# ontypehq/libfst

Hardware: AMD Instinct MI355X
Metric: strings/sec, compose_frozen_shortest_path_ambiguous len=64 batch=1M (higher is better)
Workload: dtype f64; 1 GPU; compose_frozen_shortest_path_ambiguous; semantics=eager, len=64, transducer_len=4096, branches=12, strings_per_gpu=1048576, global_batch=1048576, scaling_mode=weak: 1048576 strings per GPU per step, parallelism=dp1 (string shards, rhs replicated via RCCL broadcast)

## Files before the change

### libfst_amd/csrc/code_pull.hip

```cpp
#include <algorithm>

#include "pull_kernel_dispatch.hpp"

namespace fstamd {

namespace {
const void* pull_codes_kernel_for(const DeviceFst& rhs, uint32_t max_len, bool log = false) {
  const int rk = pull_rk(rhs, max_len);
  if (rk < 2) return nullptr;
  route_rk("eager", rk, rhs.rev, log);
  if (rk == 3) {
    const bool pack = pull_pack(rhs, max_len);
    if (log && std::getenv("FSTAMD_ROUTE_LOG"))
      std::fprintf(stderr, "[libfst_amd route] eager pull: packed cells %s\n", pack ? "on" : "off");
    if (pack) return pull_kernel_for<6, false, true>(rhs.rev);
  }
  switch (rk) {
    case 5: return pull_kernel_for<5, false, true>(rhs.rev);
    case 4: return pull_kernel_for<4, false, true>(rhs.rev);
    case 3: return pull_kernel_for<3, false, true>(rhs.rev);
    default: return pull_kernel_for<2, false, true>(rhs.rev);
  }
}
}

bool pull_codes_table(const DeviceFst& rhs, int semantics, uint32_t max_len, double* table) {
  if (semantics != 1 || !rhs.pull_ok || !pull_codes_kernel_for(rhs, max_len)) return false;
  const int rk = pull_rk(rhs, max_len);
  if (rk >= 4) {
    if (rhs.wtab_host.size() != kPullWtMax) return false;
    std::copy(rhs.wtab_host.begin(), rhs.wtab_host.end(), table);
  } else {
    for (uint32_t c = 0; c < 256; ++c) table[c] = (double)c * rhs.rev.winv;
  }
  return true;
}

int code_pull_waves_per_cu(const DeviceFst& rhs, uint32_t max_len) {
  int occ = 0;
  const void* k = pull_codes_kernel_for(rhs, max_len);
  if (!k || hipOccupancyMaxActiveBlocksPerMultiprocessor(&occ, k, 64, 0) != hipSuccess) occ = 1;
  return std::max(occ, 1);
}

hipError_t launch_eager_pull_codes(const DeviceFst& rhs, const ChainInput& in, uint32_t n_best,
                                   unsigned int* next_item, const EagerLaunch& lp,
                                   const BatchOutDev& out, uint32_t grid, hipStream_t stream) {
  const void* k = pull_codes_kernel_for(rhs, in.max_len, true);
  if (!k) return hipErrorInvalidValue;
  void* args[] = {(void*)&rhs.view, (void*)&rhs.rev, (void*)&in, (void*)&n_best,
                  (void*)&next_item, (void*)&lp, (void*)&out};
  return hipLaunchKernel(k, dim3(grid), dim3(64), args, 0, stream);
}

}
```

### libfst_amd/csrc/device_engine.hpp

```cpp
#pragma once

#include <hip/hip_runtime.h>

#include <atomic>
#include <condition_variable>
#include <cstdint>
#include <functional>
#include <mutex>
#include <new>
#include <vector>

#include "fst_core.hpp"

namespace fstamd {

class FrozenFst;

constexpr uint32_t kSpanMixed = 0xFFFFFFFEu;
constexpr uint32_t kSpanNone = 0xFFFFFFFFu;
constexpr uint32_t kRecPad = 16;
constexpr uint32_t kDeadLabel = 0xFFFFFFFFu;

struct RhsView {
  const uint2* span;
  const double* final_w;
  const uint32_t* il;
  const ArcRec* rec;
  const uint4* sspan;
  uint32_t num_states;
  uint32_t num_arcs;
  uint32_t start;
  uint32_t max_span;
  uint32_t jump_back;
  uint32_t jump_fwd;
  const uint4* sspan2;
};

constexpr uint32_t kRevPos = 0x1000u;
struct RevRec {
  uint32_t src;
  uint32_t y;
  double weight;
};
static_assert(sizeof(RevRec) == 16, "RevRec is one 16-byte load");
struct RevView {
  const uint4* rspan;
  const uint4* gtab;
  const RevRec* rrec;
  const uint32_t* rolab;
  uint32_t kp;
  uint32_t gsearch;
  uint32_t direct;
  const uint4* rrec32;
  const uint2* rrec8;
  const uint32_t* rlab;
  const uint2* rxrec;
  uint32_t nrec;
  const uint32_t* rrec4;
  uint32_t rbias8;
  double winv;
};
constexpr uint32_t kPullWt = 64;
constexpr uint32_t kPullWtMax = 256;
__host__ __device__ inline const double* rv_weight_table(const RevView& rv) {
  return reinterpret_cast<const double*>(rv.rrec4 + ((rv.nrec + 1u) & ~1u));
}
__host__ __device__ inline const uint32_t* rv_packed(const RevView& rv) {
  return rv.rrec4 + ((rv.nrec + 1u) & ~1u);
}
constexpr double kRec8WMax = 7.0;

struct DeviceFst {
  int dev = 0;
  uint8_t* blob = nullptr;
  size_t blob_size = 0;
  uint2* span = nullptr;
  double* final_w = nullptr;
  uint32_t* il = nullptr;
  ArcRec* rec = nullptr;
  uint4* sspan = nullptr;
  RhsView view{};
  bool has_eps = false;
  bool nonneg = true;
  bool nan = false;
  bool finite = true;
  uint8_t weight_type = 0;
  bool pull_ok = false;
  bool lazy_pull_ok = false;
  double int_wmax = -1.0;
  bool widx = false;
  uint32_t wt_n = 0;
  bool pack = false;
  bool byte_back = false;
  std::vector<double> wtab_host;
  mutable std::atomic<int> skip_tiny_lazy{0}, skip_tiny_eager{0};
  mutable std::atomic<int> tiny_lazy_256{0}, tiny_eager_256{0};
  mutable std::atomic<uint64_t> tiny_lazy_seen{0}, tiny_lazy_over{0};
  RevView rev{};
  void* rev_bufs[9] = {};
  uint32_t* band_il = nullptr;
  ArcRec* band_rec = nullptr;
  uint32_t band_sh = 0;
  bool band_ol_sorted = false;
  std::vector<uint32_t> perm;

  static DeviceFst* create(const FrozenFst& f, int dev);
  static DeviceFst* adopt(const void* d_blob, const FrozenFst& host_view, int dev);
  static void destroy(DeviceFst* d);
};

struct BatchOutDev {
  int32_t* status;
  uint32_t* path_len;
  uint64_t* path_off;
  double* final_w;
  uint32_t* out_il;
  uint32_t* out_ol;
  double* out_w;
  uint64_t arc_cap;
  unsigned long long* cursor;
  uint32_t* work;
  const uint64_t* slots = nullptr;
  uint32_t* host_ol = nullptr;
  union {
    double* host_w = nullptr;
    const struct TextOutDev* text;
    const struct LatticeOutDev* lattice;
  };
  int32_t* first_status = nullptr;
};

constexpr uint32_t kTextNotBytes = 0xFFFFFFFFu;
struct TextOutDev {
  uint8_t* host_text;
  uint32_t* nbytes;
  double* total_w;
};

struct LatItem {
  uint64_t spos, apos;
  uint32_t n, a;
  uint32_t pad[2];
};
static_assert(sizeof(LatItem) == 32, "two 16-B stores per item");
struct LatticeOutDev {
// ... 524 lines not shown
```

### libfst_amd/csrc/eager_pull.hip

```cpp
#include <algorithm>
#include <cmath>
#include <cstdio>
#include <cstdlib>
#include <cstring>
#include <unordered_map>
#include <vector>

#include "device_engine.hpp"
#include "host_fst.hpp"
#include "kernels/pull_window.hpp"
#include "pull_kernel_dispatch.hpp"

namespace fstamd {


void free_reverse_mirror(DeviceFst* d) {
  for (void*& p : d->rev_bufs) {
    if (p) (void)hipFree(p);
    p = nullptr;
  }
  d->rev = RevView{};
  d->pull_ok = false;
  d->widx = false;
  d->wt_n = 0;
  d->wtab_host.clear();
  d->pack = false;
}

bool build_reverse_mirror(DeviceFst* d, const FrozenFst& f) {
  d->pull_ok = false;
  d->lazy_pull_ok = false;
  if (std::getenv("FSTAMD_NO_PULL")) return true;
  if (d->has_eps || !d->nonneg || d->nan) return true;
  const uint32_t ns = f.num_states(), na = f.header().num_arcs;
  if (ns == 0 || ns >= (1u << 27)) return true;
  const StateEntry* se = f.states();
  const PackedArc* pa = f.arcs();
  const std::vector<uint32_t>& perm = d->perm;
  auto pid = [&](uint32_t s) { return perm.empty() ? s : perm[s]; };

  std::vector<uint8_t> jpos(na);
  std::vector<uint32_t> src(na);
  std::vector<uint32_t> indeg(ns + 1, 0);
  for (uint32_t s = 0; s < ns; ++s) {
    uint32_t run = se[s].arc_offset;
    for (uint32_t a = se[s].arc_offset; a < se[s].arc_offset + se[s].num_arcs; ++a) {
      if (a > se[s].arc_offset && pa[a].ilabel != pa[a - 1].ilabel) run = a;
      if (a - run >= 8) return true;
      jpos[a] = (uint8_t)(a - run);
      src[a] = pid(s);
      ++indeg[pid(pa[a].nextstate)];
    }
  }
  bool ol_ordered = true;
  for (uint32_t s = 0; s < ns && ol_ordered; ++s)
    for (uint32_t a = se[s].arc_offset; a < se[s].arc_offset + se[s].num_arcs && ol_ordered; ++a)
      for (uint32_t b = a - jpos[a]; b < a; ++b)
        if (pa[b].nextstate == pa[a].nextstate && pa[b].olabel > pa[a].olabel) {
          ol_ordered = false;
          break;
        }
  std::vector<uint32_t> ioff(ns + 1, 0);
  for (uint32_t t = 0; t < ns; ++t) ioff[t + 1] = ioff[t] + indeg[t];
  std::vector<uint32_t> in(na), fill(ioff.begin(), ioff.end() - 1);
  for (uint32_t a = 0; a < na; ++a) in[fill[pid(pa[a].nextstate)]++] = a;
  for (uint32_t t = 0; t < ns; ++t)
    std::sort(in.begin() + ioff[t], in.begin() + ioff[t + 1], [&](uint32_t x, uint32_t y) {
      if (pa[x].ilabel != pa[y].ilabel) return pa[x].ilabel < pa[y].ilabel;
      if (src[x] != src[y]) return src[x] < src[y];
      return jpos[x] < jpos[y];
    });
  struct Group { uint32_t t, label, first, n; };
  std::vector<Group> groups;
  for (uint32_t t = 0; t < ns; ++t)
    for (uint32_t i = ioff[t]; i < ioff[t + 1];) {
      uint32_t e = i + 1;
      while (e < ioff[t + 1] && pa[in[e]].ilabel == pa[in[i]].ilabel) ++e;
      groups.push_back(Group{t, pa[in[i]].ilabel, i, e - i});
      i = e;
// ... 126 lines not shown
  };
  std::vector<uint32_t> rrec4;
  uint32_t rbias8 = 0;
  int64_t dlo = 0, dhi = 0;
  if (!rrec8.empty() || widx) {
    for (size_t r = 0; r < rrec.size(); ++r) {
      if (rrec[r].src == 0xFFFFFFF8u) continue;
      const int64_t dl = (int64_t)rtgt[r] - (int64_t)(rrec[r].src >> 3);
      dlo = std::min(dlo, dl);
      dhi = std::max(dhi, dl);
    }
    if ((dhi - dlo) * 8 < 0xFFF0 && -dlo * 8 + 8 * (int64_t)kPullW <= 0xFFFF && byte_back) {
      rbias8 = (uint32_t)(-dlo * 8);
      rrec4.resize(rrec.size());
      for (size_t r = 0; r < rrec.size(); ++r) {
        const uint32_t y = rrec[r].y;
        if (rrec[r].src == 0xFFFFFFF8u) {
          rrec4[r] = 0xFFFF0000u;
        } else {
          const uint32_t low = (((y >> 17) & 7u) << 13) | (((y >> 13) & 15u) << 9) |
                               (((y >> 12) & 1u) << 8) | low_weight(rrec[r].weight);
          const int64_t dl = (int64_t)rtgt[r] - (int64_t)(rrec[r].src >> 3);
          rrec4[r] = ((uint32_t)((dl - dlo) * 8) << 16) | low;
        }
      }
    }
  }
  if (d->int_wmax >= 0.0) {
    rrec32.resize(rrec.size());
    for (size_t r = 0; r < rrec.size(); ++r)
      rrec32[r] = make_uint4(rrec[r].src, rrec[r].y, wsc(rrec[r].weight), rolab[r]);
  }
  bool pack = !rrec4.empty() && !widx && !rrec8.empty() && kp < 15 && rbias8 % 8 == 0;
  for (size_t g = 0; g < groups.size() && pack; ++g) pack = groups[g].label != 0xFFFFFFu;
  for (size_t r = 0; r < rrec4.size() && pack; ++r)
    pack = rrec4[r] == 0xFFFF0000u || (rrec4[r] >> 16) / 2 <= 252;
  pack = pack && pack_guards_fit((uint32_t)std::max<int64_t>(d->view.jump_back, -dlo),
                                 (uint32_t)std::max<int64_t>(d->view.jump_fwd, dhi), kPullW);
  if (pack) {
    const size_t n = rrec4.size();
    rrec4.resize(((n + 1) & ~(size_t)1) + n, 0xFFFF0000u);
    uint32_t* const rpk = rrec4.data() + ((n + 1) & ~(size_t)1);
    for (size_t r = 0; r < n; ++r) {
      const uint32_t v = rrec4[r];
      if (v == 0xFFFF0000u) {
        const size_t first = r - r % kp;
        rpk[r] = first < r && rrec4[first] != 0xFFFF0000u ? (rpk[first] & ~15u) | 15u : 15u;
      } else {
        rpk[r] = ((v >> 17) << 24) | ((v & 0xFFu) << 16) | (((v >> 13) & 7u) << 4) | ((v >> 9) & 15u);
      }
    }
  }
  d->pack = pack;
  if (rrec4.empty()) wtab.clear();
  if (!wtab.empty()) {
    d->wt_n = (uint32_t)wtab.size();
    wtab.resize(kPullWtMax, 0.0);
    d->wtab_host = wtab;
    rrec4.resize((rrec4.size() + 1) & ~(size_t)1, 0xFFFF0000u);
    const size_t at = rrec4.size();
    rrec4.resize(at + 2 * kPullWtMax);
    std::memcpy(rrec4.data() + at, wtab.data(), kPullWtMax * sizeof(double));
  }
  d->widx = !wtab.empty();
  auto up = [&](int i, const void* src_p, size_t bytes) -> bool {
    if (bytes == 0) bytes = 16;
    if (hipMalloc(&d->rev_bufs[i], bytes) != hipSuccess) return false;
    return hipMemcpy(d->rev_bufs[i], src_p, bytes, hipMemcpyHostToDevice) == hipSuccess;
  };
  const uint4 zero4 = make_uint4(0u, 0u, 0u, 0u);
  if (gtab.empty()) gtab.push_back(zero4);
  if (!up(0, rspan.data(), rspan.size() * sizeof(uint4)) ||
      !up(1, gtab.data(), gtab.size() * sizeof(uint4)) ||
      !up(2, rrec.data(), rrec.size() * sizeof(RevRec)) ||
      !up(3, rolab.data(), rolab.size() * sizeof(uint32_t)) ||
      (!rrec32.empty() && !up(4, rrec32.data(), rrec32.size() * sizeof(uint4))) ||
      (!rrec8.empty() && !up(5, rrec8.data(), rrec8.size() * sizeof(uint2))) ||
      (direct && (!up(6, rlab.data(), rlab.size() * sizeof(uint32_t)) ||
                  !up(7, rxrec.data(), rxrec.size() * sizeof(uint2)))) ||
      (!rrec4.empty() && !up(8, rrec4.data(), rrec4.size() * sizeof(uint32_t)))) {
    free_reverse_mirror(d);
    return false;
  }
  d->rev = RevView{(const uint4*)d->rev_bufs[0], (const uint4*)d->rev_bufs[1],
                   (const RevRec*)d->rev_bufs[2], (const uint32_t*)d->rev_bufs[3], kp, gsearch,
                   direct ? 1u : 0u, (const uint4*)d->rev_bufs[4], (const uint2*)d->rev_bufs[5],
                   (const uint32_t*)d->rev_bufs[6], (const uint2*)d->rev_bufs[7],
                   (uint32_t)(nblocks * kp), (const uint32_t*)d->rev_bufs[8], rbias8,
                   1.0 / wscale};
  d->byte_back = byte_back;
  d->pull_ok = true;
  d->lazy_pull_ok = ol_ordered && d->finite && !std::getenv("FSTAMD_NO_LAZY_PULL");
  return true;
}

bool pull_f32(const DeviceFst& rhs, uint32_t max_len) {
  return rhs.int_wmax >= 0.0 && rhs.rev.rrec32 && (double)max_len * rhs.int_wmax < 16777216.0;
}

int pull_waves_per_cu(const DeviceFst& rhs, uint32_t max_len) {
  int occ = 0;
  if (hipOccupancyMaxActiveBlocksPerMultiprocessor(&occ, pull_kernel_for<false>(rhs, max_len), 64, 0) !=
      hipSuccess)
    occ = 1;
  return std::max(occ, 1);
}
// ... 32 lines not shown
```

### libfst_amd/csrc/kernels/eager_pull.hpp

```cpp
#pragma once

#include <type_traits>

#include "device_common.hpp"
#include "eager_layered.hpp"
#include "eager_wave.hpp"
#include "eager_window.hpp"
#include "pull_window.hpp"

namespace fstamd {

constexpr uint32_t kPullAbsent = 0xFFFF0000u;
#ifdef FSTAMD_P_TIGHT_SELECT
constexpr bool kTightSelect = true;
#else
constexpr bool kTightSelect = false;
#endif
constexpr uint32_t kDistAbsent = 0x7F000000u;
template <typename DT>
__device__ __forceinline__ DT dist_inf() {
  if constexpr (sizeof(DT) == 4) return (DT)kDistAbsent;
  else return (DT)__builtin_huge_val();
}
template <typename DT>
__device__ __forceinline__ DT dist_min(DT a, DT b) {
  if constexpr (sizeof(DT) == 4) return min(a, b);
  else return fmin(a, b);
}


template <int W, bool F32 = false, int WT = kPullWt>
struct PullLds {
  static constexpr int kWords = W * 8 / 64;
  double d[W + 1];
  unsigned long long rk[W + 1];
  unsigned long long bits[kWords];
  uint4 pre[kWords];
  unsigned long long best;
  uint32_t bestp;
  ChaseJob job[kChaseBatch];
  double wt[WT];
};
template <int W>
struct PullLds<W, true> {
  static constexpr int kWords = W * 8 / 64;
  uint2 cell[W + 1];
  unsigned long long bits[kWords];
  uint4 pre[kWords];
  unsigned long long best;
  uint32_t bestp;
  ChaseJob job[kChaseBatch];
};

constexpr uint32_t kPackAbsent = 0x7F00FF80u;
constexpr uint32_t kPackNoRank = 0xFF80u;
constexpr uint32_t kPackPadM = 15u;
template <int W>
struct PullLdsPacked {
  static constexpr int kWords = W * 8 / 64;
  static constexpr int kCells = (int)pack_cells(W);
  static_assert(pack_guards_fit(kPackSpanMax, 0, W) && pack_guards_fit(0, kPackSpanMax, W),
                "packed cells: the guard bands hold every source of a window row");
  uint32_t cell[kCells];
  unsigned long long bits[kWords];
  uint4 pre[kWords];
  unsigned long long best;
  uint32_t bestp;
  ChaseJob job[kChaseBatch];
};
__device__ __forceinline__ uint32_t pack_candidate(uint32_t r, uint32_t c) {
  uint32_t cand;
  asm("v_mad_u32_u24 %0, %1, 1, %2" : "=v"(cand) : "v"(r), "v"(c));
  return cand;
}
__device__ __forceinline__ bool pack_counts(uint32_t cand) {
  return (cand & 0xFFFFu) < kPackNoRank && (cand & 15u) != kPackPadM;
}

template <int KP, typename DT>
__device__ __forceinline__ uint32_t tight_min(const DT (&nd)[KP], DT b, const uint32_t (&pk)[KP]) {
  uint32_t t[KP];
#pragma unroll
  for (int m = 0; m < KP; ++m) t[m] = nd[m] == b ? pk[m] : 0xFFFFFFFFu;
  uint32_t c = t[0];
#pragma unroll
  for (int m = 1; m < KP; m += 2) c = m + 1 < KP ? min(min(c, t[m]), t[m + 1]) : min(c, t[m]);
  return c;
}

template <typename T>
__device__ __forceinline__ const T* at_byte(const T* base, uint32_t byte_off) {
  return reinterpret_cast<const T*>(reinterpret_cast<const char*>(base) + byte_off);
}

template <int W>
__device__ __forceinline__ void pull_candidate(const PullLds<W>& S, const RevRec& r,
                                               uint32_t tmin8, uint32_t& pk, double& nd,
                                               uint32_t& rank_word) {
  const uint32_t off = min(r.src - tmin8, 8u * W);
  const double d = *reinterpret_cast<const double*>(reinterpret_cast<const char*>(S.d) + FB(off, 8 * (W + 1), 150));
  const uint32_t rw = *reinterpret_cast<const uint32_t*>(reinterpret_cast<const char*>(S.rk) + FB(off, 8 * (W + 1), 151));
  pk = rw | r.y | off;
  rank_word = rw;
  nd = d + r.weight;
}
template <int W, int WT>
__device__ __forceinline__ void pull_candidate(const PullLds<W, false, WT>& S, const uint32_t& r,
                                               uint32_t base8, uint32_t& pk, double& nd,
                                               uint32_t& rank_word) {
// ... 22 lines not shown
  const uint32_t off = min(r.x - tmin8, 8u * W);
  const uint2 c = *reinterpret_cast<const uint2*>(reinterpret_cast<const char*>(S.cell) + FB(off, 8 * (W + 1), 152));
  pk = c.y | r.y | off;
  rank_word = c.y;
  nd = c.x + rec8_weight(r.y);
}

template <int W>
__device__ __forceinline__ void pull_candidate(const PullLds<W, true>& S, const uint32_t& r,
                                               uint32_t base8, uint32_t& pk, uint32_t& nd,
                                               uint32_t& rank_word) {
  const uint32_t off = min(base8 - (r >> 16), 8u * W);
  const uint2 c = *reinterpret_cast<const uint2*>(reinterpret_cast<const char*>(S.cell) + FB(off, 8 * (W + 1), 152));
  pk = c.y | (r & 0xFFFFu);
  rank_word = c.y;
  nd = c.x + (r & 0xFFu);
}

__device__ __forceinline__ void pull_group(const RevView& rv, uint32_t lab, uint32_t t,
                                           uint32_t& rec0, uint32_t& nb) {
  const uint4 rs = rv.rspan[t];
  const bool hit = rs.z == lab && lab < kSpanMixed;
  rec0 = hit ? rs.x : 0u;
  nb = hit ? rs.y : 0u;
  if (rv.gsearch && __ballot(rs.z == kSpanMixed)) {
    if (rs.z == kSpanMixed) {
      uint32_t a = rs.x, b = rs.x + rs.y;
      for (uint32_t it = 0; it < rv.gsearch; ++it) {
        if (a < b) {
          const uint32_t mid = (a + b) >> 1;
          if (rv.gtab[mid].x < lab) a = mid + 1;
          else b = mid;
        }
      }
      if (a < rs.x + rs.y) {
        const uint4 g = rv.gtab[a];
        if (g.x == lab) {
          rec0 = g.y;
          nb = g.z;
        }
      }
    }
  }
}

template <int EW, int KP, bool DIRECT, int WAVES_PER_EU, int RK = 0, bool TEXT = false,
          bool CODES = false>
__global__ void __launch_bounds__(64, WAVES_PER_EU)
eager_pull_kernel(RhsView rhs, RevView rv, ChainInput in, uint32_t n_best,
                  unsigned int* next_item, EagerLaunch lp, BatchOutDev out) {
  constexpr int W = 64 * EW;
  constexpr bool F32 = RK != 0 && RK != 4 && RK != 5;
  constexpr bool REC4 = RK >= 3;
  constexpr bool PACK = RK == 6;
  static_assert(!PACK || (DIRECT && KP < (int)kPackPadM), "packed cells: direct layout, m = 15 is padding");
  static_assert(!CODES || (RK >= 2 && RK <= 6 && !TEXT), "weight codes: byte-weight records, label batches");
  constexpr int WT = RK == 5 ? (int)kPullWtMax : (int)kPullWt;
  using DT = typename std::conditional<F32, uint32_t, double>::type;
  using RT = typename std::conditional<
      REC4, uint32_t,
      typename std::conditional<RK == 2, uint2,
                                typename std::conditional<F32, uint4, RevRec>::type>::type>::type;
  constexpr uint32_t kRankShift = PACK ? 7 : REC4 ? 16 : 20;
  constexpr uint32_t kFirstShift = kRankShift - 3;
  constexpr uint32_t kMShift = kFirstShift - 4;
  using LdsT = typename std::conditional<PACK, PullLdsPacked<W>, PullLds<W, F32, WT>>::type;
  constexpr int kWords = LdsT::kWords;
  constexpr uint32_t kAbsent = PACK ? kPackNoRank : kPullAbsent;
  static_assert(KP <= 16, "m is 4 bits of the key");
  static_assert(W < 512, "8 * slot is 12 bits of the key, ranks 9 bits");
  __shared__ LdsT S;
  const uint32_t lane = threadIdx.x;
  const DT kInf = PACK ? (DT)(kPackAbsent >> 16) : dist_inf<DT>();
  const uint32_t* const rpk = PACK ? rv_packed(rv) : nullptr;
  auto set_cell = [&](uint32_t i, DT d, uint32_t rw) {
    if constexpr (PACK) {
      S.cell[FB(kPackGuardLo + i, LdsT::kCells, 153)] = ((uint32_t)d << 16) | rw;
    } else if constexpr (F32) {
      S.cell[FB(i, W + 1, 153)] = make_uint2(d, rw);
    } else {
      S.d[FB(i, W + 1, 154)] = d;
      S.rk[FB(i, W + 1, 155)] = rw;
    }
  };
  auto rec = [&](uint32_t r) -> RT {
    if constexpr (PACK) return rpk[r];
    else if constexpr (REC4) return rv.rrec4[r];
    else if constexpr (RK == 2) return rv.rrec8[r];
    else if constexpr (F32) return rv.rrec32[r];
    else return rv.rrec[r];
  };
  uint2* const slabs = lp.back_ws + (size_t)blockIdx.x * kChaseBatch * lp.back_cap;
  uint32_t njobs = 0;

  auto chase_batch = [&]() {
    wave_lds_sync();
    uint32_t maxL = 0;
    ChaseJob jb{};
    if (lane < njobs) {
      jb = S.job[FB(lane, kChaseBatch, 156)];
      maxL = jb.L;
    }
    maxL = __builtin_amdgcn_readfirstlane(__ockl_wfred_max_u32(maxL));
    const uint32_t* sl = reinterpret_cast<const uint32_t*>(slabs + (size_t)lane * lp.back_cap);
    const uint2* hdr = slabs + (size_t)lane * lp.back_cap + lp.back_cap / 2;
    uint32_t id = jb.id;
    uint32_t tcur = jb.pad;
    for (uint32_t t = 0; t < maxL; ++t) {
      if (lane < njobs && t < jb.L) {
        const uint32_t k = jb.L - 1 - t;
        uint32_t b;
        if constexpr (REC4) {
          const uint32_t v = reinterpret_cast<const uint8_t*>(sl)[FB(id, lp.back_cap, 60)];
          b = FB(v < (uint32_t)KP ? tcur * KP + v : rv.rxrec[tcur].x + v - KP, rv.nrec, 63);
        } else {
          b = FB(sl[FB(id, lp.back_cap, 60)], rv.nrec, 63);
        }
        const uint2 h = hdr[k];
        if constexpr (!TEXT)
          if (!out.host_ol) out.out_il[jb.o + k] = in.labels[jb.off + k];
        uint32_t src8;
        if constexpr (PACK) {
          const uint32_t r = rpk[b];
          out.out_ol[jb.o + k] = rv.rolab[b];
          if constexpr (CODES)
            reinterpret_cast<uint8_t*>(out.out_w)[jb.o + k] = (uint8_t)(r >> 16);
          else
// ... 60 lines not shown
    asm volatile("" : "+s"(w));
    return w != 0u;
  };

  if constexpr (PACK) {
#pragma unroll 1
    for (uint32_t i = lane; i < (uint32_t)LdsT::kCells; i += 64)
      S.cell[FB(i, LdsT::kCells, 153)] = kPackAbsent;
  } else {
#pragma unroll 1
  for (uint32_t i = lane; i < (uint32_t)W + 1; i += 64) set_cell(i, kInf, kAbsent);
  }
  if (lane < (uint32_t)kWords) S.bits[FB(lane, kWords, 157)] = 0;
  if constexpr (RK == 4 || RK == 5)
    for (uint32_t i = lane; i < (uint32_t)WT; i += 64) S.wt[i] = rv_weight_table(rv)[i];
  wave_lds_sync();
  uint32_t wlast = 0;

  for (;;) {
    uint32_t item = 0;
    if (lane == 0) item = atomicAdd(next_item, 1u);
    item = __builtin_amdgcn_readfirstlane(item);
    if (item >= num_items) break;
    const uint32_t si = __builtin_amdgcn_readfirstlane(lp.items ? lp.items[item] : item);
    uint32_t* const back = reinterpret_cast<uint32_t*>(slabs + (size_t)njobs * lp.back_cap);
    uint2* const hdr = slabs + (size_t)njobs * lp.back_cap + lp.back_cap / 2;
    const uint64_t off0 = in.offsets[si];
    const uint64_t off = ((uint64_t)__builtin_amdgcn_readfirstlane((uint32_t)(off0 >> 32)) << 32) |
                         __builtin_amdgcn_readfirstlane((uint32_t)off0);
    const uint32_t L = __builtin_amdgcn_readfirstlane((uint32_t)(in.offsets[si + 1] - off));

    if (rhs.start == kNoState || n_best != 1) {
      if (lane == 0)
        write_status(out, si, (rhs.start == kNoState || n_best == 0) ? kPathEmpty : kPathErrorN,
                     0, 0);
      continue;
    }
    const unsigned long long t0 = __builtin_amdgcn_s_memrealtime();

#pragma unroll 1
    for (uint32_t i = lane; i < wlast; i += 64) set_cell(i, kInf, kAbsent);
    wave_lds_sync();
    if (lane == 0) set_cell(0, (DT)w_one(), 0u);
    wave_lds_sync();
    uint32_t tmin = rhs.start, wk = 1, base = 0, n_cur = 1;
    uint32_t cmin = rhs.start, cmax = rhs.start;
    uint32_t tuples = 1, relax = 0;
    int32_t fail = F32 && L > in.max_len ? kPathOverflow : kPathOk;
    unsigned long long mykey = kMaxU64;
    uint32_t myp = kEmptyKey;
    double myfw = 0.0;

    uint32_t labs = 0;
    for (uint32_t k = 0; k < L && fail == kPathOk; ++k) {
      if ((k & 15u) == 0 && __builtin_amdgcn_s_memrealtime() - t0 > lp.wd_ticks) {
        fail = kPathInternal;
        break;
      }
      if constexpr (TEXT) {
        if ((k & 63u) == 0) labs = k + lane < L ? in.text[off + k + lane] + 1u : 0u;
      } else
      if ((k & 63u) == 0) labs = k + lane < L ? in.labels[off + k + lane] : 0u;
      const uint32_t lab = __builtin_amdgcn_readlane(labs, k & 63u);
      if (lab == kEpsilon) {
        fail = kPathUnsupported;
        break;
      }
      const uint32_t tn = pull_win_tn(cmin, rhs.jump_back);
      const uint32_t hi = pull_win_hi(cmax, rhs.jump_fwd, rhs.num_states);
      const uint32_t nbase = base + wk;
      if (pull_win_overflow(tn, hi, (uint32_t)W) || nbase + pull_win_wn(tn, hi) > lp.back_cap ||
          k >= lp.back_cap / 2) {
        fail = kPathOverflow;
        break;
      }
      const uint32_t wn = pull_win_wn(tn, hi);
      const uint32_t rows_n = pull_win_rows(wn);

      uint32_t fst[EW], bk[EW], bra[EW];
      DT bd[EW];
#pragma unroll
      for (int e = 0; e < EW; ++e) {
        fst[e] = kEmptyKey;
        bk[e] = kEmptyKey;
        bra[e] = 0;
        bd[e] = kInf;
        if ((uint32_t)e >= rows_n) continue;
        const uint32_t i = (uint32_t)e * 64 + lane;
        const uint32_t t = tn + i;
        uint32_t rec0, nb, xrec = 0;
        uint32_t tmin8 = tmin << 3;
        RT rr[KP];
        if constexpr (DIRECT) {
          const uint32_t rs = *at_byte(rv.rlab, t * 4u);
          if constexpr (PACK) {
            const uint32_t* const R = at_byte(rpk, t * (4u * KP));
#pragma unroll
            for (int m = 0; m < KP; ++m) rr[m] = R[m];
            __builtin_amdgcn_sched_barrier(0);
          }
          const bool hit = (rs & 0xFFFFFFu) == lab && lab < (PACK ? 0xFFFFFFu : kSpanMixed);
          if constexpr (PACK) tmin8 = hit ? pack_hit_base4(t, tmin, rv.rbias8 >> 1) : kPackMissBase4;
          else tmin8 = hit ? tmin8 : tmin8 + 0x80000000u;
          rec0 = t * KP;
          nb = hit ? rs >> 24 : 0u;
        } else {
          pull_group(rv, lab, t, rec0, nb);
        }
        if constexpr (REC4 && !PACK) tmin8 = (t << 3) - (tmin << 3) + rv.rbias8 + (tmin8 - (tmin << 3));
        if constexpr (!PACK) {
          const RT* R;
          if constexpr (REC4) R = at_byte(rv.rrec4, rec0 * 4u);
          else if constexpr (RK == 2) R = at_byte(rv.rrec8, rec0 * 8u);
          else if constexpr (F32) R = rv.rrec32 + rec0;
          else R = rv.rrec + rec0;
#pragma unroll
          for (int m = 0; m < KP; ++m) rr[m] = R[m];
        }
        uint32_t pk[KP], rw[KP];
        DT nd[KP];
        uint32_t f = kEmptyKey;
        DT b = kInf;
        uint32_t c = kEmptyKey;
        if constexpr (PACK) {
#pragma unroll
          for (int m = 0; m < KP; ++m) {
            const uint32_t off = pack_src_off4(tmin8, rr[m] >> 24);
            rw[m] = *reinterpret_cast<const uint32_t*>(reinterpret_cast<const char*>(S.cell) + FB(off, 4 * LdsT::kCells, 152));
          }
#pragma unroll
          for (int m = 0; m < KP; ++m) pk[m] = pack_candidate(rr[m], rw[m]);
// ... 24 lines not shown
            for (int m = 0; m < KP; ++m) c = min(c, nd[m] == b ? pk[m] : kEmptyKey);
          }
          if (want_work()) {
#pragma unroll
            for (int m = 0; m < KP; ++m) relax += (uint32_t)__popcll(__ballot(rw[m] < kPullAbsent));
          }
        }
        uint32_t ra = (REC4 ? 0u : rec0) + ((c >> kMShift) & 15u);
        if (__ballot(nb > 1)) {
          if constexpr (DIRECT) {
            const uint2 xr = nb > 1 ? rv.rxrec[t] : make_uint2(0u, nb);
            xrec = xr.x;
            nb = xr.y;
          }
          for (uint32_t x = 1;; ++x) {
            const bool act = nb > x;
            if (!__ballot(act)) break;
            const uint32_t rx = act ? (DIRECT ? xrec + (x - 1) * KP : rec0 + x * KP)
                                    : (DIRECT ? rhs.num_states * KP : 0u);
#pragma unroll
            for (int m = 0; m < KP; ++m) {
              if constexpr (PACK) {
                const uint32_t r2 = rec(rx + m);
                const uint32_t off = pack_src_off4(tmin8, r2 >> 24);
                const uint32_t cl = *reinterpret_cast<const uint32_t*>(reinterpret_cast<const char*>(S.cell) + FB(off, 4 * LdsT::kCells, 152));
                const uint32_t p2 = pack_candidate(r2, cl);
                if (act) {
                  f = min(f, p2 & 0xFFFFu);
                  if (p2 < c) {
                    c = p2;
                    ra = x * KP + m;
                  }
                }
                if (want_work()) relax += (uint32_t)__popcll(__ballot(act && pack_counts(p2)));
              } else {
                uint32_t p2, w2;
                DT n2;
                pull_candidate<W>(S, rec(rx + m), tmin8, p2, n2, w2);
                f = min(f, p2);
                if (n2 < b || (n2 == b && p2 < c)) {
                  b = n2;
                  c = p2;
                  ra = REC4 ? x * KP + m : rx + m;
                }
                if (want_work()) relax += (uint32_t)__popcll(__ballot(w2 < kPullAbsent));
              }
            }
          }
        }
        fst[e] = f;
        bd[e] = b;
        bk[e] = c;
        bra[e] = ra;
        if (f < kAbsent) {
          const uint32_t key = f >> kFirstShift;
          atomicOr(reinterpret_cast<uint32_t*>(S.bits) + FB(key >> 5, 2 * kWords, 158), 1u << (key & 31u));
        }
      }
      wave_lds_sync();

      const uint32_t nw = (n_cur * 8 + 63) / 64;
      unsigned long long word = 0;
      if (lane < nw) word = S.bits[FB(lane, kWords, 159)];
      const uint32_t pc = (uint32_t)__popcll(word);
      const uint32_t inc = wave_incl_scan_dpp(pc);
      const uint32_t n_next = __builtin_amdgcn_readlane(inc, 63);
      if (lane < nw) {
        S.pre[FB(lane, kWords, 160)] = make_uint4(inc - pc, (uint32_t)word,
                                 inc - pc + (uint32_t)__popc((uint32_t)word), (uint32_t)(word >> 32));
        S.bits[FB(lane, kWords, 161)] = 0;
      }
      wave_lds_sync();
      if (n_next == 0) {
        n_cur = 0;
        break;
      }

      const bool last = k + 1 == L;
      if (lane == 0) hdr[k] = make_uint2(base, tmin);
      const uint32_t rows_w = max(rows_n, (wk + 63) / 64);
      uint32_t lo_slot = kEmptyKey, hi_slot = 0;
#pragma unroll
      for (int e = 0; e < EW; ++e) {
        if ((uint32_t)e >= rows_w) continue;
        const uint32_t i = (uint32_t)e * 64 + lane;
        if ((uint32_t)e >= rows_n) {
          set_cell(i, bd[e], kAbsent);
          continue;
        }
        uint32_t fe = fst[e];
        asm volatile("" : "+v"(fe));
        const bool pres = fe < kAbsent;
        const uint32_t key = pres ? fe >> kFirstShift : 0u;
        const uint2 p = reinterpret_cast<const uint2*>(S.pre)[FB(key >> 5, 2 * kWords, 162)];
        const uint32_t rank = p.x + (uint32_t)__popc(p.y & ((1u << (key & 31u)) - 1u));
        if constexpr (PACK)
          S.cell[FB(kPackGuardLo + i, LdsT::kCells, 153)] = (bk[e] & 0xFFFF0000u) | (pres ? rank << kRankShift : kAbsent);
        else
          set_cell(i, bd[e], pres ? rank << kRankShift : kPullAbsent);
        const unsigned long long pm = __ballot(pres);
        if (pm) {
          lo_slot = min(lo_slot, (uint32_t)e * 64 + (uint32_t)__builtin_ctzll(pm));
          hi_slot = max(hi_slot, (uint32_t)e * 64 + 63u - (uint32_t)__builtin_clzll(pm));
        }
        if (pres) {
          if constexpr (REC4)
            reinterpret_cast<uint8_t*>(back)[FB(nbase + i, lp.back_cap, 61)] = (uint8_t)bra[e];
          else
            *const_cast<uint32_t*>(at_byte(back, FB(nbase + i, lp.back_cap, 61) * 4u)) = bra[e];
          if (last) {
            const uint32_t t = tn + i;
            const double fw2 = rhs.final_w[FB(t, rhs.num_states, 62)];
            const DT de = PACK ? (DT)(bk[e] >> 16) : bd[e];
            if (!w_is_zero((double)de) && !w_is_zero(fw2)) {
              const unsigned long long kk = okey((double)de * (F32 ? rv.winv : 1.0) + fw2);
              const uint32_t pp = (rank << 9) | i;
              if (kk < mykey || (kk == mykey && pp < myp)) {
                mykey = kk;
                myp = pp;
                myfw = fw2;
              }
            }
          }
        }
      }
      tmin = tn;
      base = nbase;
      wk = wn;
      n_cur = n_next;
      tuples += n_next;
      cmin = tn + lo_slot;
      cmax = tn + hi_slot;
      wave_lds_sync();
    }
    wlast = wk;

    if (fail != kPathOk) {
      if (lane == 0) write_status(out, si, fail, tuples, relax);
      continue;
    }
    if (L == 0 && lane == 0) {
      const double fw2 = rhs.final_w[rhs.start];
      if (!w_is_zero(fw2)) {
        mykey = okey(w_one() + fw2);
        myp = 0;
        myfw = fw2;
      }
    }
// ... 33 lines not shown
```

### libfst_amd/csrc/pull_kernel_dispatch.hpp

```cpp
#pragma once

#include <cstdio>
#include <cstdlib>

#include "device_engine.hpp"
#include "kernels/eager_pull.hpp"
#include "kernels/lazy_pull.hpp"

namespace fstamd {

namespace {

template <int KP, int WV, int RK, bool TEXT, bool CODES = false>
const void* pull_kernel_ptr(bool direct) {
  return direct ? (const void*)eager_pull_kernel<kPullRows, KP, true, WV, RK, TEXT, CODES>
                : (const void*)eager_pull_kernel<kPullRows, KP, false, WV, RK, TEXT, CODES>;
}
#ifndef FSTAMD_PULL_WAVES_SMALL
#define FSTAMD_PULL_WAVES_SMALL 5
#endif
#ifndef FSTAMD_PULL_WAVES_F32
#define FSTAMD_PULL_WAVES_F32 6
#endif
#ifndef FSTAMD_PULL_WAVES_R8
#define FSTAMD_PULL_WAVES_R8 7
#endif
#ifndef FSTAMD_PULL_WAVES_PACK
#define FSTAMD_PULL_WAVES_PACK FSTAMD_PULL_WAVES_R8
#endif
template <int RK, bool TEXT, bool CODES = false>
const void* pull_kernel_for(const RevView& rv) {
  const bool dir = rv.direct != 0;
  if constexpr (RK == 6) {
    switch (rv.kp) {
      case 4: return (const void*)eager_pull_kernel<kPullRows, 4, true, FSTAMD_PULL_WAVES_PACK, 6, TEXT, CODES>;
      case 5: return (const void*)eager_pull_kernel<kPullRows, 5, true, FSTAMD_PULL_WAVES_PACK, 6, TEXT, CODES>;
      default: return (const void*)eager_pull_kernel<kPullRows, 8, true, 4, 6, TEXT, CODES>;
    }
  } else {
    constexpr int wv = RK == 5 ? 4
                     : RK == 4 ? FSTAMD_PULL_WAVES_SMALL
                     : RK >= 2 ? FSTAMD_PULL_WAVES_R8 : RK ? FSTAMD_PULL_WAVES_F32 : FSTAMD_PULL_WAVES_SMALL;
    switch (rv.kp) {
      case 4: return pull_kernel_ptr<4, wv, RK, TEXT, CODES>(dir);
      case 5: return pull_kernel_ptr<5, wv, RK, TEXT, CODES>(dir);
      default: return pull_kernel_ptr<8, 4, RK, TEXT, CODES>(dir);
    }
  }
}
bool use_rec8(const RevView& rv) { return rv.rrec8 && !std::getenv("FSTAMD_NO_REC8"); }
int route_rk(const char* sem, int rk, const RevView& rv, bool log) {
  if (log && std::getenv("FSTAMD_ROUTE_LOG"))
    std::fprintf(stderr, "[libfst_amd route] %s pull: records %d, weight scale %g\n", sem, rk,
                 rk && rk < 4 ? 1.0 / rv.winv : 1.0);
  return rk;
}
int pull_rk(const DeviceFst& rhs, uint32_t max_len) {
  if (!pull_f32(rhs, max_len) || std::getenv("FSTAMD_P_F64"))
    return rhs.rev.rrec4 && rhs.widx && !std::getenv("FSTAMD_NO_REC4")
               ? (rhs.wt_n <= kPullWt ? 4 : 5)
               : 0;
  if (rhs.rev.rrec4 && use_rec8(rhs.rev) && !std::getenv("FSTAMD_NO_REC4")) return 3;
  return use_rec8(rhs.rev) ? 2 : 1;
}
bool pull_pack(const DeviceFst& rhs, uint32_t max_len) {
  return rhs.pack && pull_rk(rhs, max_len) == 3 &&
         ((double)max_len + 1.0) * rhs.int_wmax < (double)0x7F00 && !std::getenv("FSTAMD_NO_PACK");
}
template <bool TEXT>
const void* pull_kernel_for(const DeviceFst& rhs, uint32_t max_len, bool log = false) {
  const int rk = route_rk("eager", pull_rk(rhs, max_len), rhs.rev, log);
  if (rk == 3) {
    const bool pack = pull_pack(rhs, max_len);
    if (log && std::getenv("FSTAMD_ROUTE_LOG"))
      std::fprintf(stderr, "[libfst_amd route] eager pull: packed cells %s\n", pack ? "on" : "off");
    if (pack) return pull_kernel_for<6, TEXT>(rhs.rev);
  }
  switch (rk) {
    case 0: return pull_kernel_for<0, TEXT>(rhs.rev);
    case 5: return pull_kernel_for<5, TEXT>(rhs.rev);
    case 4: return pull_kernel_for<4, TEXT>(rhs.rev);
    case 3: return pull_kernel_for<3, TEXT>(rhs.rev);
    case 2: return pull_kernel_for<2, TEXT>(rhs.rev);
    default: return pull_kernel_for<1, TEXT>(rhs.rev);
  }
}
#ifndef FSTAMD_LP_WAVES_F32
#define FSTAMD_LP_WAVES_F32 5
#endif
#ifndef FSTAMD_LP_WAVES_F64
#define FSTAMD_LP_WAVES_F64 4
#endif
constexpr int kLazyPullWaves = 3;
template <int KP, int RK, bool TEXT>
const void* lazy_pull_ptr(bool direct, bool b1) {
  constexpr int wv = KP > 5 ? kLazyPullWaves
                   : RK ? FSTAMD_LP_WAVES_F32 : FSTAMD_LP_WAVES_F64;
  if (!direct) return (const void*)lazy_pull_kernel<kPullRows, KP, false, wv, RK, false, TEXT>;
  return b1 ? (const void*)lazy_pull_kernel<kPullRows, KP, true, wv, RK, true, TEXT>
            : (const void*)lazy_pull_kernel<kPullRows, KP, true, wv, RK, false, TEXT>;
}
template <int RK, bool TEXT>
const void* lazy_pull_kernel_for(const DeviceFst& rhs) {
  const bool dir = rhs.rev.direct != 0, b1 = dir && rhs.byte_back;
  switch (rhs.rev.kp) {
    case 4: return lazy_pull_ptr<4, RK, TEXT>(dir, b1);
    case 5: return lazy_pull_ptr<5, RK, TEXT>(dir, b1);
    default: return lazy_pull_ptr<8, RK, TEXT>(dir, b1);
  }
}
template <bool TEXT>
const void* lazy_pull_kernel_for(const DeviceFst& rhs, uint32_t max_len, bool log = false) {
  const int rk = !lazy_pull_f32(rhs, max_len) ? 0 : use_rec8(rhs.rev) ? 2 : 1;
  if (log && std::getenv("FSTAMD_ROUTE_LOG"))
    std::fprintf(stderr, "[libfst_amd route] lazy pull: back records %d B\n",
                 rhs.rev.direct && rhs.byte_back ? 1 : 4);
  switch (route_rk("lazy", rk, rhs.rev, log)) {
    case 0: return lazy_pull_kernel_for<0, TEXT>(rhs);
    case 2: return lazy_pull_kernel_for<2, TEXT>(rhs);
    default: return lazy_pull_kernel_for<1, TEXT>(rhs);
  }
}
}

}
```

Baseline: 41.34 million strings/s.

## Add ordered-layer fast path skipping frontier bitset compaction in packed eager pull

Adds a host-side analysis that marks states whose same-label arc runs reach contiguous, monotone target ranges. It also builds a next-bad-state table that the kernel reads per step. When the current frontier window holds only conforming states, the packed pull kernel uses the cell index as rank and counts survivors with a ballot popcount. This skips the LDS atomicOr bitset, the prefix scan and the extra wave sync. The cost is an extra scalar load per step, a new kernel variant and more code complexity, and correctness depends on the conformance analysis being right.

```diff
diff --git a/libfst_amd/csrc/code_pull.hip b/libfst_amd/csrc/code_pull.hip
--- a/libfst_amd/csrc/code_pull.hip
+++ b/libfst_amd/csrc/code_pull.hip
@@ -13,7 +13,9 @@
     const bool pack = pull_pack(rhs, max_len);
     if (log && std::getenv("FSTAMD_ROUTE_LOG"))
       std::fprintf(stderr, "[libfst_amd route] eager pull: packed cells %s\n", pack ? "on" : "off");
-    if (pack) return pull_kernel_for<6, false, true>(rhs.rev);
+    if (pack)
+      return pull_ordered(rhs, log) ? pull_kernel_for<7, false, true>(rhs.rev)
+                                    : pull_kernel_for<6, false, true>(rhs.rev);
   }
   switch (rk) {
     case 5: return pull_kernel_for<5, false, true>(rhs.rev);
diff --git a/libfst_amd/csrc/device_engine.hpp b/libfst_amd/csrc/device_engine.hpp
--- a/libfst_amd/csrc/device_engine.hpp
+++ b/libfst_amd/csrc/device_engine.hpp
@@ -67,6 +67,9 @@
 }
 __host__ __device__ inline const uint32_t* rv_packed(const RevView& rv) {
   return rv.rrec4 + ((rv.nrec + 1u) & ~1u);
+}
+__host__ __device__ inline const uint32_t* rv_nextbad(const RevView& rv) {
+  return rv_packed(rv) + rv.nrec;
 }
 constexpr double kRec8WMax = 7.0;
 
@@ -91,6 +94,7 @@
   bool widx = false;
   uint32_t wt_n = 0;
   bool pack = false;
+  bool ordered = false;
   bool byte_back = false;
   std::vector<double> wtab_host;
   mutable std::atomic<int> skip_tiny_lazy{0}, skip_tiny_eager{0};
diff --git a/libfst_amd/csrc/eager_pull.hip b/libfst_amd/csrc/eager_pull.hip
--- a/libfst_amd/csrc/eager_pull.hip
+++ b/libfst_amd/csrc/eager_pull.hip
@@ -8,6 +8,7 @@
 
 #include "device_engine.hpp"
 #include "host_fst.hpp"
+#include "kernels/pull_ordered.hpp"
 #include "kernels/pull_window.hpp"
 #include "pull_kernel_dispatch.hpp"
 
@@ -25,6 +26,7 @@
   d->wt_n = 0;
   d->wtab_host.clear();
   d->pack = false;
+  d->ordered = false;
 }
 
 bool build_reverse_mirror(DeviceFst* d, const FrozenFst& f) {
@@ -257,6 +259,40 @@
     }
   }
   d->pack = pack;
+  d->ordered = false;
+  if (pack) {
+    std::vector<uint32_t> order(ns);
+    for (uint32_t s = 0; s < ns; ++s) order[pid(s)] = s;
+    std::vector<uint8_t> bad(ns, 0);
+    std::unordered_map<uint32_t, uint32_t> lo_of;
+    uint32_t nconf = 0, first_bad = ns;
+    for (uint32_t ds = 0; ds < ns; ++ds) {
+      const uint32_t s = order[ds];
+      const uint32_t a0 = se[s].arc_offset, a1 = a0 + se[s].num_arcs;
+      for (uint32_t a = a0; a < a1;) {
+        uint32_t tg[8], n = 0;
+        uint32_t e = a;
+        for (; e < a1 && pa[e].ilabel == pa[a].ilabel; ++e) tg[n++] = pid(pa[e].nextstate);
+        const auto it = lo_of.find(pa[a].ilabel);
+        uint32_t lo;
+        if (!ordered_run_conforms(tg, n, it == lo_of.end() ? kOrderedNoPrev : it->second, &lo))
+          bad[ds] = 1;
+        lo_of[pa[a].ilabel] = lo;
+        a = e;
+      }
+      if (bad[ds]) first_bad = std::min(first_bad, ds);
+      else ++nconf;
+    }
+    d->ordered = nconf > 0;
+    const size_t at = rrec4.size();
+    rrec4.resize(at + ordered_table_words(ns));
+    ordered_fill_nextbad(bad.data(), ns, rrec4.data() + at);
+    if (std::getenv("FSTAMD_ROUTE_LOG"))
+      std::fprintf(stderr,
+                   "[libfst_amd route] eager pull: ordered layers %s, %u of %u states conforming, "
+                   "first non-conforming %u\n",
+                   d->ordered ? "on" : "off", nconf, ns, first_bad);
+  }
   if (rrec4.empty()) wtab.clear();
   if (!wtab.empty()) {
     d->wt_n = (uint32_t)wtab.size();
diff --git a/libfst_amd/csrc/kernels/eager_pull.hpp b/libfst_amd/csrc/kernels/eager_pull.hpp
--- a/libfst_amd/csrc/kernels/eager_pull.hpp
+++ b/libfst_amd/csrc/kernels/eager_pull.hpp
@@ -6,6 +6,7 @@
 #include "eager_layered.hpp"
 #include "eager_wave.hpp"
 #include "eager_window.hpp"
+#include "pull_ordered.hpp"
 #include "pull_window.hpp"
 
 namespace fstamd {
@@ -55,6 +56,10 @@
 constexpr uint32_t kPackAbsent = 0x7F00FF80u;
 constexpr uint32_t kPackNoRank = 0xFF80u;
 constexpr uint32_t kPackPadM = 15u;
+constexpr uint32_t kPackDistAbsent = kPackAbsent >> 16;
+static_assert((kPackAbsent & 0xFFFF0000u) == (kPackDistAbsent << 16) &&
+                  2ull * kPackDistAbsent <= 0x10000ull,
+              "packed cells: an absent distance field plus a launch's weights stays in 16 bits");
 template <int W>
 struct PullLdsPacked {
   static constexpr int kWords = W * 8 / 64;
@@ -183,9 +188,11 @@
   constexpr int W = 64 * EW;
   constexpr bool F32 = RK != 0 && RK != 4 && RK != 5;
   constexpr bool REC4 = RK >= 3;
-  constexpr bool PACK = RK == 6;
+  constexpr bool PACK = RK == 6 || RK == 7;
+  constexpr bool ORD = RK == 7;
   static_assert(!PACK || (DIRECT && KP < (int)kPackPadM), "packed cells: direct layout, m = 15 is padding");
-  static_assert(!CODES || (RK >= 2 && RK <= 6 && !TEXT), "weight codes: byte-weight records, label batches");
+  static_assert(!ORD || (uint32_t)(64 * EW - 1) << 7 < kPackNoRank, "ordered layers: a slot fits the rank field");
+  static_assert(!CODES || (RK >= 2 && RK <= 7 && !TEXT), "weight codes: byte-weight records, label batches");
   constexpr int WT = RK == 5 ? (int)kPullWtMax : (int)kPullWt;
   using DT = typename std::conditional<F32, uint32_t, double>::type;
   using RT = typename std::conditional<
@@ -204,6 +211,8 @@
   const uint32_t lane = threadIdx.x;
   const DT kInf = PACK ? (DT)(kPackAbsent >> 16) : dist_inf<DT>();
   const uint32_t* const rpk = PACK ? rv_packed(rv) : nullptr;
+  using CU32 = const __attribute__((address_space(4))) uint32_t;
+  CU32* const nextbad = ORD ? (CU32*)rv_nextbad(rv) : nullptr;
   auto set_cell = [&](uint32_t i, DT d, uint32_t rw) {
     if constexpr (PACK) {
       S.cell[FB(kPackGuardLo + i, LdsT::kCells, 153)] = ((uint32_t)d << 16) | rw;
@@ -370,6 +379,7 @@
     double myfw = 0.0;
 
     uint32_t labs = 0;
+    uint32_t ordered = ORD ? 1u : 0u;
     for (uint32_t k = 0; k < L && fail == kPathOk; ++k) {
       if ((k & 15u) == 0 && __builtin_amdgcn_s_memrealtime() - t0 > lp.wd_ticks) {
         fail = kPathInternal;
@@ -384,6 +394,8 @@
         fail = kPathUnsupported;
         break;
       }
+      [[maybe_unused]] uint32_t nbad = 0;
+      if constexpr (ORD) nbad = nextbad[FB(cmin, ordered_table_words(rhs.num_states), 164)];
       const uint32_t tn = pull_win_tn(cmin, rhs.jump_back);
       const uint32_t hi = pull_win_hi(cmax, rhs.jump_fwd, rhs.num_states);
       const uint32_t nbase = base + wk;
@@ -394,7 +406,11 @@
       }
       const uint32_t wn = pull_win_wn(tn, hi);
       const uint32_t rows_n = pull_win_rows(wn);
-
+      if constexpr (ORD)
+        if (ordered) ordered = ordered_layer_ok(nbad, cmax) ? 1u : 0u;
+
+      const bool ob = ORD && ordered != 0u;
+      uint32_t n_next = 0;
       uint32_t fst[EW], bk[EW], bra[EW];
       DT bd[EW];
 #pragma unroll
@@ -525,6 +541,9 @@
         bd[e] = b;
         bk[e] = c;
         bra[e] = ra;
+        if (ob) {
+          n_next += (uint32_t)__popcll(__ballot(c < (kPackDistAbsent << 16)));
+        } else
         if (f < kAbsent) {
           const uint32_t key = f >> kFirstShift;
           atomicOr(reinterpret_cast<uint32_t*>(S.bits) + FB(key >> 5, 2 * kWords, 158), 1u << (key & 31u));
@@ -532,18 +551,20 @@
       }
       wave_lds_sync();
 
-      const uint32_t nw = (n_cur * 8 + 63) / 64;
+      if (!ob) {
+      const uint32_t nw = ((ORD ? wk : n_cur) * 8 + 63) / 64;
       unsigned long long word = 0;
       if (lane < nw) word = S.bits[FB(lane, kWords, 159)];
       const uint32_t pc = (uint32_t)__popcll(word);
       const uint32_t inc = wave_incl_scan_dpp(pc);
-      const uint32_t n_next = __builtin_amdgcn_readlane(inc, 63);
+      n_next = __builtin_amdgcn_readlane(inc, 63);
       if (lane < nw) {
         S.pre[FB(lane, kWords, 160)] = make_uint4(inc - pc, (uint32_t)word,
                                  inc - pc + (uint32_t)__popc((uint32_t)word), (uint32_t)(word >> 32));
         S.bits[FB(lane, kWords, 161)] = 0;
       }
       wave_lds_sync();
+      }
       if (n_next == 0) {
         n_cur = 0;
         break;
@@ -561,12 +582,19 @@
           set_cell(i, bd[e], kAbsent);
           continue;
         }
-        uint32_t fe = fst[e];
-        asm volatile("" : "+v"(fe));
-        const bool pres = fe < kAbsent;
-        const uint32_t key = pres ? fe >> kFirstShift : 0u;
-        const uint2 p = reinterpret_cast<const uint2*>(S.pre)[FB(key >> 5, 2 * kWords, 162)];
-        const uint32_t rank = p.x + (uint32_t)__popc(p.y & ((1u << (key & 31u)) - 1u));
+        bool pres;
+        uint32_t rank;
+        if (ob) {
+          pres = bk[e] < (kPackDistAbsent << 16);
+          rank = i;
+        } else {
+          uint32_t fe = fst[e];
+          asm volatile("" : "+v"(fe));
+          pres = fe < kAbsent;
+          const uint32_t key = pres ? fe >> kFirstShift : 0u;
+          const uint2 p = reinterpret_cast<const uint2*>(S.pre)[FB(key >> 5, 2 * kWords, 162)];
+          rank = p.x + (uint32_t)__popc(p.y & ((1u << (key & 31u)) - 1u));
+        }
         if constexpr (PACK)
           S.cell[FB(kPackGuardLo + i, LdsT::kCells, 153)] = (bk[e] & 0xFFFF0000u) | (pres ? rank << kRankShift : kAbsent);
         else
diff --git a/libfst_amd/csrc/kernels/pull_ordered.hpp b/libfst_amd/csrc/kernels/pull_ordered.hpp
--- /dev/null
+++ b/libfst_amd/csrc/kernels/pull_ordered.hpp
@@ -0,0 +1,44 @@
+#pragma once
+
+#include <cstdint>
+
+#if defined(__HIP__) || defined(__CUDACC__)
+#define FSTAMD_ORD_HD __host__ __device__
+#else
+#define FSTAMD_ORD_HD
+#endif
+
+namespace fstamd {
+
+constexpr uint32_t kOrderedNoPrev = 0xFFFFFFFFu;
+
+FSTAMD_ORD_HD constexpr bool ordered_run_ok(const uint32_t* tg, uint32_t n, uint32_t* lo_out) {
+  uint32_t lo = tg[0], hi = tg[0], mn = tg[0];
+  bool ok = true;
+  for (uint32_t j = 1; j < n; ++j) {
+    const uint32_t t = tg[j];
+    if (t < mn) mn = t;
+    if (t >= lo && t <= hi) continue;
+    if (t == hi + 1) hi = t;
+    else ok = false;
+  }
+  *lo_out = mn;
+  return ok;
+}
+FSTAMD_ORD_HD constexpr bool ordered_run_conforms(const uint32_t* tg, uint32_t n, uint32_t lo_prev,
+                                                  uint32_t* lo_out) {
+  const bool ok = ordered_run_ok(tg, n, lo_out);
+  return ok && (lo_prev == kOrderedNoPrev || *lo_out >= lo_prev);
+}
+
+inline void ordered_fill_nextbad(const uint8_t* bad, uint32_t num_states, uint32_t* nextbad) {
+  nextbad[num_states] = num_states;
+  for (uint32_t s = num_states; s-- > 0;) nextbad[s] = bad[s] ? s : nextbad[s + 1];
+}
+constexpr uint32_t ordered_table_words(uint32_t num_states) { return num_states + 1; }
+
+FSTAMD_ORD_HD constexpr bool ordered_layer_ok(uint32_t nextbad_cmin, uint32_t cmax) {
+  return nextbad_cmin > cmax;
+}
+
+}
diff --git a/libfst_amd/csrc/pull_kernel_dispatch.hpp b/libfst_amd/csrc/pull_kernel_dispatch.hpp
--- a/libfst_amd/csrc/pull_kernel_dispatch.hpp
+++ b/libfst_amd/csrc/pull_kernel_dispatch.hpp
@@ -31,11 +31,11 @@
 template <int RK, bool TEXT, bool CODES = false>
 const void* pull_kernel_for(const RevView& rv) {
   const bool dir = rv.direct != 0;
-  if constexpr (RK == 6) {
+  if constexpr (RK >= 6) {
     switch (rv.kp) {
-      case 4: return (const void*)eager_pull_kernel<kPullRows, 4, true, FSTAMD_PULL_WAVES_PACK, 6, TEXT, CODES>;
-      case 5: return (const void*)eager_pull_kernel<kPullRows, 5, true, FSTAMD_PULL_WAVES_PACK, 6, TEXT, CODES>;
-      default: return (const void*)eager_pull_kernel<kPullRows, 8, true, 4, 6, TEXT, CODES>;
+      case 4: return (const void*)eager_pull_kernel<kPullRows, 4, true, FSTAMD_PULL_WAVES_PACK, RK, TEXT, CODES>;
+      case 5: return (const void*)eager_pull_kernel<kPullRows, 5, true, FSTAMD_PULL_WAVES_PACK, RK, TEXT, CODES>;
+      default: return (const void*)eager_pull_kernel<kPullRows, 8, true, 4, RK, TEXT, CODES>;
     }
   } else {
     constexpr int wv = RK == 5 ? 4
@@ -65,7 +65,13 @@
 }
 bool pull_pack(const DeviceFst& rhs, uint32_t max_len) {
   return rhs.pack && pull_rk(rhs, max_len) == 3 &&
-         ((double)max_len + 1.0) * rhs.int_wmax < (double)0x7F00 && !std::getenv("FSTAMD_NO_PACK");
+         ((double)max_len + 1.0) * rhs.int_wmax < (double)kPackDistAbsent && !std::getenv("FSTAMD_NO_PACK");
+}
+bool pull_ordered(const DeviceFst& rhs, bool log) {
+  const bool ord = rhs.ordered && !std::getenv("FSTAMD_NO_ORDERED");
+  if (log && std::getenv("FSTAMD_ROUTE_LOG"))
+    std::fprintf(stderr, "[libfst_amd route] eager pull: ordered layers %s\n", ord ? "on" : "off");
+  return ord;
 }
 template <bool TEXT>
 const void* pull_kernel_for(const DeviceFst& rhs, uint32_t max_len, bool log = false) {
@@ -74,7 +80,7 @@
     const bool pack = pull_pack(rhs, max_len);
     if (log && std::getenv("FSTAMD_ROUTE_LOG"))
       std::fprintf(stderr, "[libfst_amd route] eager pull: packed cells %s\n", pack ? "on" : "off");
-    if (pack) return pull_kernel_for<6, TEXT>(rhs.rev);
+    if (pack) return pull_ordered(rhs, log) ? pull_kernel_for<7, TEXT>(rhs.rev) : pull_kernel_for<6, TEXT>(rhs.rev);
   }
   switch (rk) {
     case 0: return pull_kernel_for<0, TEXT>(rhs.rev);
```

Measured after the change: 38.58 million strings/s. -6.7%, worse.
